# voutcn/megahit

Measured on NVIDIA H100. Metric: sorted (k+1)-mer edges/sec at k=27 on 150bp reads, higher is better.
Workload: dtype u32

## Files before the change

### megahit_b200/csrc/mhb_hashcount.cu

```cuda
#include <cuda_runtime.h>
#include <stdio.h>
#include <string.h>

#include "mhb.h"
#include "mhb_common.cuh"
#include "mhb_count.cuh"

using namespace mhb;

namespace {

constexpr int kHcHist = 1024;
constexpr u64 kHcEmpty = ~0ull;
constexpr int kHcBatch = 4;
constexpr u32 kRemBits = 42;
constexpr u32 kHcHotCount = 256;
constexpr int kHcHotRound = 32;
constexpr int kHcMaxProbes = 48;
constexpr int kHcStack = 72;

__device__ __forceinline__ u64 rec_key64(const uint2 r) { return ((u64)r.x << 32) | r.y; }

__global__ void k_bucket_bounds(const uint2 *__restrict__ recs, u64 n, u64 *__restrict__ bounds) {
  const u32 b = blockIdx.x * blockDim.x + threadIdx.x;
  if (b > 65536u) return;
  u64 lo = 0, hi = n;
  while (lo < hi) {
    const u64 mid = (lo + hi) >> 1;
    if ((recs[mid].x >> 16) < b) lo = mid + 1;
    else hi = mid;
  }
  bounds[b] = lo;
}

template <int THREADS_, int LOG_SLOTS_, int CTAS_>
struct HcGeom {
  static constexpr int THREADS = THREADS_, LOG_SLOTS = LOG_SLOTS_, SLOTS = 1 << LOG_SLOTS_, CTAS = CTAS_;
  static constexpr int MAX_SOLID = SLOTS / 4;
  static constexpr int CELLS = 2 * THREADS;
  static constexpr int LOG_CELLS = LOG_SLOTS_ - 2 >= 0 ? (THREADS_ == 256 ? 9 : (THREADS_ == 512 ? 10 : 11)) : 9;
  static constexpr u32 SLICE = (u32)(SLOTS * 1.83);
};

template <class G>
struct HcShared {
  u64 keys[G::SLOTS];
  u32 cnt[G::SLOTS];
  u32 pt[G::SLOTS];
  u32 nt[G::SLOTS];
  u64 sorted[G::MAX_SOLID];
  u64 tmp[G::MAX_SOLID];
  u32 cell_base[G::CELLS];
  u32 cell_cur[G::CELLS];
  u32 cta_hist[kHcHist];
  u32 wide[kHcHotRound][8];
  uint16_t hot_slot[G::MAX_SOLID];
  u64 st_prefix[kHcStack];
  u32 st_bits[kHcStack];
  u32 warp_sum[G::THREADS / 32];
  u32 n_solid, n_hot, overflow, bucket, out_cursor, sp;
};

__device__ __forceinline__ u32 lane_lt_mask() { return (1u << (threadIdx.x & 31)) - 1u; }

__device__ __forceinline__ void smem_add(u32 *p, u32 v) {
  asm volatile("red.shared.add.u32 [%0], %1;" ::"r"((u32)__cvta_generic_to_shared(p)), "r"(v) : "memory");
}

template <class G>
__device__ __forceinline__ u32 hc_hash(u64 r) { return (u32)((r * 0x9E3779B97F4A7C15ull) >> (64 - G::LOG_SLOTS)); }

template <class G>
__device__ __forceinline__ u32 hc_insert(HcShared<G> &s, u64 r) {
  u32 h = hc_hash<G>(r);
  for (int probes = 0; probes < kHcMaxProbes; ++probes) {
    u64 cur = s.keys[h];
    if (cur == r) return h;
    if (cur == kHcEmpty) {
      cur = atomicCAS((unsigned long long *)&s.keys[h], kHcEmpty, r);
      if (cur == kHcEmpty || cur == r) return h;
    }
    h = (h + 1) & (G::SLOTS - 1);
  }
  return G::SLOTS;
}
template <class G>
__device__ __forceinline__ u32 hc_find(const HcShared<G> &s, u64 r) {
  u32 h = hc_hash<G>(r);
  while (s.keys[h] != r) h = (h + 1) & (G::SLOTS - 1);
  return h;
}

template <class G>
__device__ __forceinline__ void hc_hist_undo(HcShared<G> &s, u64 *mul_hist) {
  for (u32 i = threadIdx.x; i < (u32)G::SLOTS; i += G::THREADS) {
    if (s.keys[i] == kHcEmpty) continue;
    const u32 c = s.cnt[i];
    const u32 c16 = c > 65535u ? 65535u : c;
    if (c16 < (u32)kHcHist) atomicAdd(&s.cta_hist[c16], 0xFFFFFFFFu);
    else atomicAdd((unsigned long long *)&mul_hist[c16], ~0ull);
  }
}

template <class G>
__device__ __forceinline__ void hc_scan_cells(HcShared<G> &s) {
  const u32 t = threadIdx.x, lane = t & 31, w = t >> 5;
  const u32 a = s.cell_base[2 * t], b = s.cell_base[2 * t + 1];
  u32 v = a + b;
#pragma unroll
  for (int d = 1; d < 32; d <<= 1) {
    const u32 o = __shfl_up_sync(0xffffffffu, v, d);
    if ((int)lane >= d) v += o;
  }
  if (lane == 31) s.warp_sum[w] = v;
  __syncthreads();
  if (w == 0) {
    u32 x = lane < G::THREADS / 32 ? s.warp_sum[lane] : 0u;
#pragma unroll
    for (int d = 1; d < 32; d <<= 1) {
      const u32 o = __shfl_up_sync(0xffffffffu, x, d);
      if ((int)lane >= d) x += o;
    }
    if (lane < G::THREADS / 32) s.warp_sum[lane] = x;
  }
  __syncthreads();
  const u32 excl = v - (a + b) + (w ? s.warp_sum[w - 1] : 0u);
  s.cell_base[2 * t] = excl;
  s.cell_base[2 * t + 1] = excl + a;
  s.cell_cur[2 * t] = excl;
  s.cell_cur[2 * t + 1] = excl + a;
  __syncthreads();
}

__device__ __forceinline__ bool hc_any_byte_ge(u32 w, u32 m) {
  return (w & 0xFFu) >= m || ((w >> 8) & 0xFFu) >= m || ((w >> 16) & 0xFFu) >= m || (w >> 24) >= m;
}

template <int THREADS>
__device__ __forceinline__ u64 hc_align(const uint2 *__restrict__ recs, u64 p, u64 lo, u64 hi, u32 *s_min) {
  if (p <= lo) return lo;
  if (p >= hi) return hi;
  for (u64 q0 = p; q0 < hi; q0 += THREADS) {
    __syncthreads();
    if (threadIdx.x == 0) *s_min = 0xFFFFFFFFu;
    __syncthreads();
    const u64 q = q0 + threadIdx.x;
    if (q < hi && (recs[q].x >> 8) != (recs[q - 1].x >> 8)) atomicMin(s_min, threadIdx.x);
    __syncthreads();
    const u32 f = *s_min;
    if (f != 0xFFFFFFFFu) return q0 + f;
  }
  return hi;
}

template <class G>
__global__ void __launch_bounds__(G::THREADS, G::CTAS)
    k_hash_count(const uint2 *__restrict__ recs, const u64 *__restrict__ bounds, const u64 *__restrict__ slice_off,
                 const u64 *__restrict__ n_slices_dev, int m, u32 *ticket, u64 *__restrict__ list,
                 u32 *__restrict__ slice_count, u64 *__restrict__ slice_base, u32 *__restrict__ slice_bucket, u64 *mul_hist,
                 u32 *err_flag) {
  constexpr int THREADS = G::THREADS, SLOTS = G::SLOTS, MAX_SOLID = G::MAX_SOLID, CELLS = G::CELLS;
  extern __shared__ __align__(16) unsigned char smem_raw[];
  HcShared<G> &s = *reinterpret_cast<HcShared<G> *>(smem_raw);
  const u32 tid = threadIdx.x;
  for (u32 i = tid; i < kHcHist; i += THREADS) s.cta_hist[i] = 0;
  for (u32 i = tid; i < (u32)SLOTS; i += THREADS) {
    s.keys[i] = kHcEmpty;
    s.cnt[i] = 0;
    s.pt[i] = 0;
    s.nt[i] = 0;
  }
  __syncthreads();
  const u64 n_slices = *n_slices_dev;
  const u32 um = (u32)m;
  while (true) {
    if (tid == 0) {
      const u32 sl = atomicAdd(ticket, 1u);
      s.bucket = sl;
      if (sl < n_slices) {
        u32 a = 0, z = 65536;
        while (z - a > 1) {
          const u32 mid = (a + z) >> 1;
          if (slice_off[mid] <= sl) a = mid; else z = mid;
        }
        s.sp = a;
      }
    }
    __syncthreads();
    const u32 sl = s.bucket;
    if (sl >= n_slices) break;
    const u32 b = s.sp;
    __syncthreads();
    const u64 blo = bounds[b], bhi = bounds[b + 1];
    const u64 n_in_b = slice_off[b + 1] - slice_off[b], idx = sl - slice_off[b];
    const u64 step = (bhi - blo + n_in_b - 1) / n_in_b;
    const u64 lo = hc_align<THREADS>(recs, blo + idx * step, blo, bhi, &s.overflow);
    const u64 hi = idx + 1 == n_in_b ? bhi : hc_align<THREADS>(recs, blo + (idx + 1) * step, blo, bhi, &s.overflow);
    __syncthreads();
    const u64 base = lo / (u64)m + sl;
    if (tid == 0) {
      slice_base[sl] = base;
      slice_bucket[sl] = b;
      s.out_cursor = 0;
      s.st_prefix[0] = 0;
      s.st_bits[0] = 0;
      s.sp = 1;
    }
    if (hi <= lo) {
      if (tid == 0) slice_count[sl] = 0;
      __syncthreads();
      continue;
    }
    __syncthreads();
    while (s.sp > 0) {
      const u32 sp = s.sp - 1;
      const u64 prefix = s.st_prefix[sp];
      const u32 bits = s.st_bits[sp];
      __syncthreads();
      if (tid == 0) {
        s.sp = sp;
        s.n_solid = 0;
        s.n_hot = 0;
        s.overflow = 0;
      }
      __syncthreads();
      for (u64 i0 = lo + tid; i0 < hi; i0 += (u64)THREADS * kHcBatch) {
        uint2 v[kHcBatch];
#pragma unroll
        for (int j = 0; j < kHcBatch; ++j) {
          const u64 i = i0 + (u64)j * THREADS;
          v[j] = i < hi ? recs[i] : make_uint2(0, 0);
        }
#pragma unroll
        for (int j = 0; j < kHcBatch; ++j) {
          const u64 i = i0 + (u64)j * THREADS;
          if (i >= hi) break;
          const u64 key = rec_key64(v[j]);
          const u64 r = (key >> 6) & ((1ull << kRemBits) - 1);
          if (bits && (r >> (kRemBits - bits)) != prefix) continue;
          const u32 h = hc_insert<G>(s, r);
          if (h == (u32)SLOTS) {
            s.overflow = 1;
            continue;
          }
          smem_add(&s.cnt[h], 1u);
          const u32 p = (u32)(key >> 3) & 7u, nx = (u32)key & 7u;
          if (p < 4) smem_add(&s.pt[h], 1u << (8 * p));
          if (nx < 4) smem_add(&s.nt[h], 1u << (8 * nx));
        }
        if (s.overflow) break;
      }
      __syncthreads();
      bool failed = s.overflow != 0;
      u32 ns = 0;
      if (!failed) {
        for (u32 i0 = 0; i0 < (u32)SLOTS; i0 += THREADS) {
          const u32 slot = i0 + tid;
          const bool on = s.keys[slot] != kHcEmpty;
          const u32 c = on ? s.cnt[slot] : 0u;
          const u32 c16 = c > 65535u ? 65535u : c;
          const u32 ones = __ballot_sync(0xffffffffu, on && c16 == 1u), twos = __ballot_sync(0xffffffffu, on && c16 == 2u);
          if (on && c16 > 2u) {
            if (c16 < (u32)kHcHist) smem_add(&s.cta_hist[c16], 1u);
            else atomicAdd((unsigned long long *)&mul_hist[c16], 1ull);
          }
          const bool solid = on && c >= um;
          const u32 sm_ = __ballot_sync(0xffffffffu, solid);
          u32 wbase = 0;
          if ((tid & 31) == 0) {
            if (ones) atomicAdd(&s.cta_hist[1], (u32)__popc(ones));
            if (twos) atomicAdd(&s.cta_hist[2], (u32)__popc(twos));
            if (sm_) wbase = atomicAdd(&s.n_solid, (u32)__popc(sm_));
          }
          wbase = __shfl_sync(0xffffffffu, wbase, 0);
          if (solid) {
            const u32 rank = wbase + __popc(sm_ & lane_lt_mask());
            if (rank < (u32)MAX_SOLID) {
              u64 e = (s.keys[slot] << 22) | ((u64)c16 << 6);
              if (c >= kHcHotCount) {
                const u32 hi_ = atomicAdd(&s.n_hot, 1u);
                if (hi_ < (u32)MAX_SOLID) s.hot_slot[hi_] = (uint16_t)slot;
                s.pt[slot] = hi_;
                s.nt[slot] = rank;
              } else {
                e |= (hc_any_byte_ge(s.pt[slot], um) ? 0ull : 1ull) | (hc_any_byte_ge(s.nt[slot], um) ? 0ull : 2ull);
              }
              s.sorted[rank] = e;
            }
          }
        }
        __syncthreads();
        ns = s.n_solid;
        if (ns > (u32)MAX_SOLID) {
          hc_hist_undo<G>(s, mul_hist);
          failed = true;
        }
      }
      if (!failed && ns) {
        const u32 n_hot = s.n_hot;
        for (u32 h0 = 0; h0 < n_hot; h0 += kHcHotRound) {
          for (u32 i = tid; i < (u32)kHcHotRound * 8; i += THREADS) s.wide[i >> 3][i & 7] = 0;
          __syncthreads();
          for (u64 i0 = lo + tid; i0 < hi; i0 += (u64)THREADS * kHcBatch) {
            uint2 v[kHcBatch];
#pragma unroll
            for (int j = 0; j < kHcBatch; ++j) {
              const u64 i = i0 + (u64)j * THREADS;
              v[j] = i < hi ? recs[i] : make_uint2(0, 0);
            }
#pragma unroll
            for (int j = 0; j < kHcBatch; ++j) {
              const u64 i = i0 + (u64)j * THREADS;
              if (i >= hi) break;
              const u64 key = rec_key64(v[j]);
              const u64 r = (key >> 6) & ((1ull << kRemBits) - 1);
              if (bits && (r >> (kRemBits - bits)) != prefix) continue;
              const u32 slot = hc_find<G>(s, r);
              const u32 c = s.cnt[slot];
              if (c < kHcHotCount || c < um) continue;
              const u32 hidx = s.pt[slot] - h0;
              if (hidx >= (u32)kHcHotRound) continue;
              const u32 p = (u32)(key >> 3) & 7u, nx = (u32)key & 7u;
              if (p < 4) smem_add(&s.wide[hidx][p], 1u);
              if (nx < 4) smem_add(&s.wide[hidx][4 + nx], 1u);
            }
          }
          __syncthreads();
          for (u32 i = tid; i < (u32)kHcHotRound && h0 + i < n_hot; i += THREADS) {
            bool has_in = false, has_out = false;
#pragma unroll
            for (int c = 0; c < 4; ++c) {
              has_in = has_in || s.wide[i][c] >= um;
              has_out = has_out || s.wide[i][4 + c] >= um;
            }
            s.sorted[s.nt[s.hot_slot[h0 + i]]] |= (has_in ? 0ull : 1ull) | (has_out ? 0ull : 2ull);
          }
          __syncthreads();
        }
        for (u32 i = tid; i < (u32)CELLS; i += THREADS) s.cell_base[i] = 0;
        __syncthreads();
        const u32 cshift = 22 + (kRemBits - G::LOG_CELLS);
        for (u32 i = tid; i < ns; i += THREADS) smem_add(&s.cell_base[(u32)((s.sorted[i] << bits) >> cshift)], 1u);
        __syncthreads();
        hc_scan_cells<G>(s);
        for (u32 i = tid; i < ns; i += THREADS) {
          const u64 e = s.sorted[i];
          s.tmp[atomicAdd(&s.cell_cur[(u32)((e << bits) >> cshift)], 1u)] = e;
        }
        __syncthreads();
        const u32 at = s.out_cursor;
        for (u32 i = tid; i < ns; i += THREADS) {
          const u64 e = s.tmp[i];
          const u32 c = (u32)((e << bits) >> cshift);
          const u32 b0 = s.cell_base[c], b1 = c + 1 < (u32)CELLS ? s.cell_base[c + 1] : ns;
          u32 r = b0;
          for (u32 j = b0; j < b1; ++j) r += s.tmp[j] < e ? 1u : 0u;
          list[base + at + r] = e;
        }
        __syncthreads();
        if (tid == 0) s.out_cursor = at + ns;
      }
      for (u32 i = tid; i < (u32)SLOTS; i += THREADS) {
        s.keys[i] = kHcEmpty;
        s.cnt[i] = 0;
        s.pt[i] = 0;
        s.nt[i] = 0;
      }
      __syncthreads();
      if (tid == 0 && failed) {
        if (bits + 2 > kRemBits || s.sp + 4 > (u32)kHcStack) atomicExch(err_flag, 1u);
        else
          for (int c = 3; c >= 0; --c) {
            s.st_prefix[s.sp] = (prefix << 2) | (u64)c;
            s.st_bits[s.sp] = bits + 2;
            ++s.sp;
          }
      }
      __syncthreads();
    }
    if (tid == 0) slice_count[sl] = s.out_cursor;
    __syncthreads();
  }
  for (u32 i = tid; i < kHcHist; i += THREADS)
    if (s.cta_hist[i]) atomicAdd((unsigned long long *)&mul_hist[i], (unsigned long long)s.cta_hist[i]);
}

using HcGeomA = HcGeom<256, 11, 3>;
using HcGeomB = HcGeom<512, 12, 2>;
using HcGeomC = HcGeom<1024, 13, 1>;

__global__ void k_slice_counts(const u64 *__restrict__ bounds, u32 T, u32 *__restrict__ cnt) {
  const u32 b = blockIdx.x * blockDim.x + threadIdx.x;
  if (b >= 65536u) return;
  const u64 nb = bounds[b + 1] - bounds[b];
  cnt[b] = (u32)((nb + T - 1) / T);
}

__global__ void __launch_bounds__(256)
    k_hash_gather(const u64 *__restrict__ list, const u64 *__restrict__ n_slices_dev, const u32 *__restrict__ slice_count,
                  const u64 *__restrict__ slice_dst, const u64 *__restrict__ slice_base, const u32 *__restrict__ slice_bucket,
                  u32 we, u32 *__restrict__ edges, uint8_t *__restrict__ aux, u64 capacity, const u32 *err_flag,
                  u64 *n_solid_out) {
  const u32 lane = threadIdx.x & 31;
  if (blockIdx.x == 0 && threadIdx.x == 0 && *err_flag) *n_solid_out = ~0ull;
  const u64 n_slices = *n_slices_dev;
  for (u64 sl = (u64)blockIdx.x * 8 + (threadIdx.x >> 5); sl < n_slices; sl += (u64)gridDim.x * 8) {
    const u32 cnt = slice_count[sl];
    if (!cnt) continue;
    const u64 base = slice_base[sl], off = slice_dst[sl], b = slice_bucket[sl];
    for (u32 x = lane; x < cnt; x += 32) {
      if (off + x >= capacity) break;
      const u64 ent = list[base + x];
      const u64 key = (b << 48) | ((ent >> 22) << 6);
      u32 *e = edges + (off + x) * we;
      e[0] = (u32)(key >> 32);
      e[1] = (u32)key;
      if (we == 3) e[2] = 0;
      e[we - 1] |= (u32)(ent >> 6) & 0xFFFFu;
      aux[off + x] = (uint8_t)(ent & 3u);
    }
  }
}

int scan_counts(cudaStream_t st, const u32 *in, u64 n, u64 *out, u64 *total_dev, u64 *bsum) {
  const u64 nb = (n + kScanTile - 1) / kScanTile;
  k_scan32_sums<<<(unsigned)nb, kScanThreads, 0, st>>>(in, n, bsum);
  CK_LAUNCH();
  k_scan_u64<<<1, 1024, 0, st>>>(bsum, nb, total_dev);
  CK_LAUNCH();
  k_scan32_apply<<<(unsigned)nb, kScanThreads, 0, st>>>(in, n, bsum, out);
  CK_LAUNCH();
  return MHB_OK;
}

static int hc_geom() {
  static const int g = getenv("MHB_HC_GEOM") ? (getenv("MHB_HC_GEOM")[0] == 'A' ? 0 : (getenv("MHB_HC_GEOM")[0] == 'C' ? 2 : 1)) : 1;
  return g;
}
static u32 hc_slice_records() {
  const u32 def = hc_geom() == 0 ? HcGeomA::SLICE : (hc_geom() == 1 ? HcGeomB::SLICE : HcGeomC::SLICE);
  static const u32 v = getenv("MHB_HC_SLICE") ? (u32)atoi(getenv("MHB_HC_SLICE")) : 0;
  return v >= 256 && v <= 64000 ? v : def;
}
#define kHcSliceRecords hc_slice_records()

template <class G>
static int launch_hash_count(cudaStream_t st, const uint2 *recs, const u64 *bounds, const u64 *slice_off, const u64 *n_slices_dev,
                             int m, u32 *misc, u64 *list, u32 *slice_count, u64 *slice_base, u32 *slice_bucket, u64 *mul_hist) {
  static int bps = 0;
  const size_t smem = sizeof(HcShared<G>);
  if (!bps) {
    CK(cudaFuncSetAttribute(k_hash_count<G>, cudaFuncAttributeMaxDynamicSharedMemorySize, (int)smem));
    CK(cudaOccupancyMaxActiveBlocksPerMultiprocessor(&bps, k_hash_count<G>, G::THREADS, smem));
    if (bps < 1) return mhb_set_error(MHB_ERR_CUDA, "hash-count kernel does not fit an SM (%zu B shared memory)", smem);
    if (getenv("MHB_VERBOSE")) fprintf(stderr, "[mhb] hash count: %d threads, %d slots, %zu B smem, %d CTA/SM, slice %u\n", G::THREADS, G::SLOTS, smem, bps, kHcSliceRecords);
  }
  k_hash_count<G><<<sm_count() * bps, G::THREADS, smem, st>>>(recs, bounds, slice_off, n_slices_dev, m, misc, list, slice_count,
                                                             slice_base, slice_bucket, mul_hist, misc + 1);
  CK_LAUNCH();
  return MHB_OK;
}

struct HcLayout {
  size_t sort_ws, off_bounds, off_bcnt, off_soff, off_bsum, off_misc, off_scount, off_sdst, off_sbase, off_sbucket, off_list, total;
  uint64_t max_slices;
};
HcLayout hc_layout(uint64_t n, int32_t m) {
  HcLayout L;
  auto pad = [](size_t x) { return (x + 255) & ~(size_t)255; };
  L.max_slices = n / 256 + 65536 + 2;
  L.sort_ws = pad(mhb_sort_workspace_bytes(n, 2));
  size_t p = L.sort_ws;
  L.off_bounds = p;
  p += pad(65537 * 8);
  L.off_bcnt = p;
  p += pad(65537 * 4);
  L.off_soff = p;
  p += pad(65537 * 8);
  L.off_bsum = p;
  p += pad((L.max_slices / kScanTile + 4) * 8);
  L.off_misc = p;
  p += 256;
  L.off_scount = p;
  p += pad(L.max_slices * 4);
  L.off_sdst = p;
  p += pad(L.max_slices * 8);
  L.off_sbase = p;
  p += pad(L.max_slices * 8);
  L.off_sbucket = p;
  p += pad(L.max_slices * 4);
  L.off_list = p;
  p += pad((size_t)(n / (uint64_t)(m < 1 ? 1 : m) + L.max_slices + 8) * 8);
  L.total = p;
  return L;
}

}

extern "C" int mhb_count_hashed_supported(uint32_t k, int32_t m) {
  return count_record_words(k) == 2 && 2 * (k + 1) >= 24 && m >= 1 && m <= kHcHist;
}

extern "C" size_t mhb_count_hashed_workspace_bytes(uint64_t n, uint32_t k, int32_t m) {
  (void)k;
  return hc_layout(n, m).total;
}

extern "C" int mhb_count_solid_hashed(void *stream, uint32_t *recs_a, uint32_t *recs_b, uint64_t n, uint32_t k, int32_t m,
                                      const uint64_t *hist_byte5, uint32_t *edges_out, uint8_t *aux_out,
                                      uint64_t capacity_edges, uint64_t *mul_hist, uint64_t *n_solid_out, void *ws,
                                      size_t ws_bytes) {
  if (!mhb_count_hashed_supported(k, m)) return mhb_set_error(MHB_ERR_ARG, "hashed count needs 8-byte records (11 <= k <= 28) and 1 <= m <= %d", kHcHist);
  if (!mul_hist || !n_solid_out || !ws) return mhb_set_error(MHB_ERR_ARG, "bad args");
  if (n == 0) return MHB_OK;
  if (n >= (1ull << 40)) return mhb_set_error(MHB_ERR_ARG, "too many records for one hashed count call");
  const HcLayout L = hc_layout(n, m);
  if (ws_bytes < L.total) return mhb_set_error(MHB_ERR_ARG, "hashed count workspace too small (%zu < %zu)", ws_bytes, L.total);
  cudaStream_t st = (cudaStream_t)stream;
  const uint8_t bytes[3] = {5, 6, 7};
  int in_b = 0;
  if (int rc = mhb_sort_records_impl(st, recs_a, recs_b, n, 2, bytes, 3, hist_byte5, ws, L.sort_ws, &in_b, nullptr)) return rc;
  const uint2 *recs = (const uint2 *)(in_b ? recs_b : recs_a);
  char *w = (char *)ws;
  u64 *bounds = (u64 *)(w + L.off_bounds);
  u32 *bcnt = (u32 *)(w + L.off_bcnt);
  u64 *slice_off = (u64 *)(w + L.off_soff);
  u64 *bsum = (u64 *)(w + L.off_bsum);
  u32 *misc = (u32 *)(w + L.off_misc);
  u32 *slice_count = (u32 *)(w + L.off_scount);
  u64 *slice_dst = (u64 *)(w + L.off_sdst);
  u64 *slice_base = (u64 *)(w + L.off_sbase);
  u32 *slice_bucket = (u32 *)(w + L.off_sbucket);
  u64 *list = (u64 *)(w + L.off_list);
  u64 *n_slices_dev = (u64 *)(misc + 2);
  CK(cudaMemsetAsync(misc, 0, 256, st));
  CK(cudaMemsetAsync(slice_count, 0, L.max_slices * 4, st));
  k_bucket_bounds<<<(65537 + 255) / 256, 256, 0, st>>>(recs, n, bounds);
  CK_LAUNCH();
  k_slice_counts<<<65536 / 256, 256, 0, st>>>(bounds, kHcSliceRecords, bcnt);
  CK_LAUNCH();
  if (int rc = scan_counts(st, bcnt, 65536, slice_off, n_slices_dev, bsum)) return rc;
  CK(cudaMemcpyAsync(slice_off + 65536, n_slices_dev, 8, cudaMemcpyDeviceToDevice, st));
  {
    int rc;
    if (hc_geom() == 0) rc = launch_hash_count<HcGeomA>(st, recs, bounds, slice_off, n_slices_dev, m, misc, list, slice_count, slice_base, slice_bucket, mul_hist);
    else if (hc_geom() == 2) rc = launch_hash_count<HcGeomC>(st, recs, bounds, slice_off, n_slices_dev, m, misc, list, slice_count, slice_base, slice_bucket, mul_hist);
    else rc = launch_hash_count<HcGeomB>(st, recs, bounds, slice_off, n_slices_dev, m, misc, list, slice_count, slice_base, slice_bucket, mul_hist);
    if (rc) return rc;
  }
  if (int rc = scan_counts(st, slice_count, L.max_slices, slice_dst, n_solid_out, bsum)) return rc;
  k_hash_gather<<<sm_count() * 4, 256, 0, st>>>(list, n_slices_dev, slice_count, slice_dst, slice_base, slice_bucket,
                                               words_per_edge(k), edges_out, aux_out, capacity_edges, misc + 1, n_solid_out);
  CK_LAUNCH();
  return MHB_OK;
}
```

Measured before the change: 13.68 billion.

## Precompute slice plan, prefetch next slice to L2, and streamline hash-count loop

Slice boundary alignment moves out of the hash-count kernel into a separate per-bucket planning kernel that uses binary search. The count kernel now reads precomputed ranges, fetches the next ticket early and issues bulk L2 prefetches for the next slice while the current one is processed. Table clearing is folded into the extraction pass, and cell histogramming moves into solid extraction. Hot-key passes use a small rehash, the histogram-undo pass is dropped in favour of a done flag on the stack, the batch size doubles, and the alternative geometries and env knobs are removed. The aim is fewer block-wide syncs and less memory latency, but the kernel is more complex and register pressure may rise.

```diff
diff --git a/megahit_b200/csrc/mhb_hashcount.cu b/megahit_b200/csrc/mhb_hashcount.cu
--- a/megahit_b200/csrc/mhb_hashcount.cu
+++ b/megahit_b200/csrc/mhb_hashcount.cu
@@ -12,12 +12,14 @@
 
 constexpr int kHcHist = 1024;
 constexpr u64 kHcEmpty = ~0ull;
-constexpr int kHcBatch = 4;
+constexpr int kHcBatch = 8;
 constexpr u32 kRemBits = 42;
 constexpr u32 kHcHotCount = 256;
 constexpr int kHcHotRound = 32;
 constexpr int kHcMaxProbes = 48;
 constexpr int kHcStack = 72;
+constexpr u32 kHcHistDone = 1u << 31;
+constexpr u32 kHcPrefetchChunk = 16384;
 
 __device__ __forceinline__ u64 rec_key64(const uint2 r) { return ((u64)r.x << 32) | r.y; }
 
@@ -31,6 +33,36 @@
     else hi = mid;
   }
   bounds[b] = lo;
+}
+
+__device__ __forceinline__ u64 hc_align(const uint2 *__restrict__ recs, u64 p, u64 lo, u64 hi) {
+  if (p <= lo) return lo;
+  if (p >= hi) return hi;
+  const u32 pre = recs[p - 1].x >> 8;
+  u64 a = p, z = hi;
+  while (a < z) {
+    const u64 mid = (a + z) >> 1;
+    if ((recs[mid].x >> 8) > pre) z = mid;
+    else a = mid + 1;
+  }
+  return a;
+}
+
+__global__ void k_slice_plan(const uint2 *__restrict__ recs, const u64 *__restrict__ bounds, const u64 *__restrict__ slice_off,
+                             int m, ulonglong2 *__restrict__ plan, u64 *__restrict__ slice_base, u32 *__restrict__ slice_bucket) {
+  const u32 b = blockIdx.x * blockDim.x + threadIdx.x;
+  if (b >= 65536u) return;
+  const u64 s0 = slice_off[b], ns = slice_off[b + 1] - s0;
+  if (!ns) return;
+  const u64 blo = bounds[b], bhi = bounds[b + 1], step = (bhi - blo + ns - 1) / ns;
+  u64 lo = blo;
+  for (u64 i = 0; i < ns; ++i) {
+    const u64 hi = i + 1 == ns ? bhi : hc_align(recs, blo + (i + 1) * step, blo, bhi);
+    plan[s0 + i] = make_ulonglong2(lo, hi);
+    slice_base[s0 + i] = lo / (u64)m + s0 + i;
+    slice_bucket[s0 + i] = b;
+    lo = hi;
+  }
 }
 
 template <int THREADS_, int LOG_SLOTS_, int CTAS_>
@@ -54,17 +86,27 @@
   u32 cell_cur[G::CELLS];
   u32 cta_hist[kHcHist];
   u32 wide[kHcHotRound][8];
-  uint16_t hot_slot[G::MAX_SOLID];
+  uint16_t hot_rank[G::MAX_SOLID];
   u64 st_prefix[kHcStack];
   u32 st_bits[kHcStack];
   u32 warp_sum[G::THREADS / 32];
-  u32 n_solid, n_hot, overflow, bucket, out_cursor, sp;
+  ulonglong2 nx_range[2];
+  u32 nx_sl[2];
+  u32 n_solid[2], n_hot[2], overflow[2];
 };
 
 __device__ __forceinline__ u32 lane_lt_mask() { return (1u << (threadIdx.x & 31)) - 1u; }
 
 __device__ __forceinline__ void smem_add(u32 *p, u32 v) {
   asm volatile("red.shared.add.u32 [%0], %1;" ::"r"((u32)__cvta_generic_to_shared(p)), "r"(v) : "memory");
+}
+
+__device__ __forceinline__ void hc_prefetch_l2(const uint2 *recs, u64 lo, u64 hi) {
+  const u64 a0 = (u64)(recs + lo) & ~15ull, a1 = (u64)(recs + hi) & ~15ull;
+  for (u64 a = a0; a < a1; a += kHcPrefetchChunk) {
+    const u32 sz = (u32)(a1 - a < kHcPrefetchChunk ? a1 - a : kHcPrefetchChunk);
+    asm volatile("cp.async.bulk.prefetch.L2.global [%0], %1;" ::"l"(a), "r"(sz) : "memory");
+  }
 }
 
 template <class G>
@@ -85,27 +127,20 @@
   return G::SLOTS;
 }
 template <class G>
-__device__ __forceinline__ u32 hc_find(const HcShared<G> &s, u64 r) {
+__device__ __forceinline__ u32 hc_lookup(const HcShared<G> &s, u64 r) {
   u32 h = hc_hash<G>(r);
-  while (s.keys[h] != r) h = (h + 1) & (G::SLOTS - 1);
-  return h;
-}
-
-template <class G>
-__device__ __forceinline__ void hc_hist_undo(HcShared<G> &s, u64 *mul_hist) {
-  for (u32 i = threadIdx.x; i < (u32)G::SLOTS; i += G::THREADS) {
-    if (s.keys[i] == kHcEmpty) continue;
-    const u32 c = s.cnt[i];
-    const u32 c16 = c > 65535u ? 65535u : c;
-    if (c16 < (u32)kHcHist) atomicAdd(&s.cta_hist[c16], 0xFFFFFFFFu);
-    else atomicAdd((unsigned long long *)&mul_hist[c16], ~0ull);
+  while (true) {
+    const u64 cur = s.keys[h];
+    if (cur == r) return h;
+    if (cur == kHcEmpty) return G::SLOTS;
+    h = (h + 1) & (G::SLOTS - 1);
   }
 }
 
 template <class G>
 __device__ __forceinline__ void hc_scan_cells(HcShared<G> &s) {
   const u32 t = threadIdx.x, lane = t & 31, w = t >> 5;
-  const u32 a = s.cell_base[2 * t], b = s.cell_base[2 * t + 1];
+  const u32 a = s.cell_cur[2 * t], b = s.cell_cur[2 * t + 1];
   u32 v = a + b;
 #pragma unroll
   for (int d = 1; d < 32; d <<= 1) {
@@ -136,94 +171,74 @@
   return (w & 0xFFu) >= m || ((w >> 8) & 0xFFu) >= m || ((w >> 16) & 0xFFu) >= m || (w >> 24) >= m;
 }
 
-template <int THREADS>
-__device__ __forceinline__ u64 hc_align(const uint2 *__restrict__ recs, u64 p, u64 lo, u64 hi, u32 *s_min) {
-  if (p <= lo) return lo;
-  if (p >= hi) return hi;
-  for (u64 q0 = p; q0 < hi; q0 += THREADS) {
-    __syncthreads();
-    if (threadIdx.x == 0) *s_min = 0xFFFFFFFFu;
-    __syncthreads();
-    const u64 q = q0 + threadIdx.x;
-    if (q < hi && (recs[q].x >> 8) != (recs[q - 1].x >> 8)) atomicMin(s_min, threadIdx.x);
-    __syncthreads();
-    const u32 f = *s_min;
-    if (f != 0xFFFFFFFFu) return q0 + f;
-  }
-  return hi;
-}
-
 template <class G>
 __global__ void __launch_bounds__(G::THREADS, G::CTAS)
-    k_hash_count(const uint2 *__restrict__ recs, const u64 *__restrict__ bounds, const u64 *__restrict__ slice_off,
-                 const u64 *__restrict__ n_slices_dev, int m, u32 *ticket, u64 *__restrict__ list,
-                 u32 *__restrict__ slice_count, u64 *__restrict__ slice_base, u32 *__restrict__ slice_bucket, u64 *mul_hist,
-                 u32 *err_flag) {
+    k_hash_count(const uint2 *__restrict__ recs, const ulonglong2 *__restrict__ plan, const u64 *__restrict__ n_slices_dev,
+                 int m, u32 *ticket, u64 *__restrict__ list, u32 *__restrict__ slice_count, u64 *mul_hist, u32 *err_flag) {
   constexpr int THREADS = G::THREADS, SLOTS = G::SLOTS, MAX_SOLID = G::MAX_SOLID, CELLS = G::CELLS;
   extern __shared__ __align__(16) unsigned char smem_raw[];
   HcShared<G> &s = *reinterpret_cast<HcShared<G> *>(smem_raw);
   const u32 tid = threadIdx.x;
   for (u32 i = tid; i < kHcHist; i += THREADS) s.cta_hist[i] = 0;
+  for (u32 i = tid; i < (u32)CELLS; i += THREADS) s.cell_cur[i] = 0;
   for (u32 i = tid; i < (u32)SLOTS; i += THREADS) {
     s.keys[i] = kHcEmpty;
     s.cnt[i] = 0;
     s.pt[i] = 0;
     s.nt[i] = 0;
   }
-  __syncthreads();
   const u64 n_slices = *n_slices_dev;
   const u32 um = (u32)m;
-  while (true) {
-    if (tid == 0) {
-      const u32 sl = atomicAdd(ticket, 1u);
-      s.bucket = sl;
-      if (sl < n_slices) {
-        u32 a = 0, z = 65536;
-        while (z - a > 1) {
-          const u32 mid = (a + z) >> 1;
-          if (slice_off[mid] <= sl) a = mid; else z = mid;
-        }
-        s.sp = a;
+  const u32 cshift = 22 + (kRemBits - G::LOG_CELLS);
+  u32 tk = 0;
+  if (tid == 0) {
+    s.n_solid[0] = s.n_solid[1] = s.n_hot[0] = s.n_hot[1] = s.overflow[0] = s.overflow[1] = 0;
+    const u32 t0 = atomicAdd(ticket, 1u);
+    s.nx_sl[0] = t0;
+    if (t0 < n_slices) {
+      const ulonglong2 r = plan[t0];
+      s.nx_range[0] = r;
+      hc_prefetch_l2(recs, r.x, r.y);
+      tk = atomicAdd(ticket, 1u);
+    } else {
+      tk = t0;
+    }
+  }
+  __syncthreads();
+  u32 q = 0;
+  for (u32 it = 0;; ++it) {
+    const u32 sl = s.nx_sl[it & 1];
+    if (sl >= n_slices) break;
+    const ulonglong2 rg = s.nx_range[it & 1];
+    const u64 lo = rg.x, hi = rg.y;
+    ulonglong2 nx = make_ulonglong2(0, 0);
+    u32 ntk = tk;
+    if (tid == 0 && tk < n_slices) {
+      nx = plan[tk];
+      ntk = atomicAdd(ticket, 1u);
+    }
+    auto publish_next = [&]() {
+      if (tid != 0) return;
+      s.nx_sl[(it + 1) & 1] = tk;
+      if (tk < n_slices) {
+        s.nx_range[(it + 1) & 1] = nx;
+        hc_prefetch_l2(recs, nx.x, nx.y);
       }
-    }
-    __syncthreads();
-    const u32 sl = s.bucket;
-    if (sl >= n_slices) break;
-    const u32 b = s.sp;
-    __syncthreads();
-    const u64 blo = bounds[b], bhi = bounds[b + 1];
-    const u64 n_in_b = slice_off[b + 1] - slice_off[b], idx = sl - slice_off[b];
-    const u64 step = (bhi - blo + n_in_b - 1) / n_in_b;
-    const u64 lo = hc_align<THREADS>(recs, blo + idx * step, blo, bhi, &s.overflow);
-    const u64 hi = idx + 1 == n_in_b ? bhi : hc_align<THREADS>(recs, blo + (idx + 1) * step, blo, bhi, &s.overflow);
-    __syncthreads();
-    const u64 base = lo / (u64)m + sl;
-    if (tid == 0) {
-      slice_base[sl] = base;
-      slice_bucket[sl] = b;
-      s.out_cursor = 0;
-      s.st_prefix[0] = 0;
-      s.st_bits[0] = 0;
-      s.sp = 1;
-    }
+      tk = ntk;
+    };
     if (hi <= lo) {
-      if (tid == 0) slice_count[sl] = 0;
+      publish_next();
       __syncthreads();
       continue;
     }
-    __syncthreads();
-    while (s.sp > 0) {
-      const u32 sp = s.sp - 1;
-      const u64 prefix = s.st_prefix[sp];
-      const u32 bits = s.st_bits[sp];
-      __syncthreads();
-      if (tid == 0) {
-        s.sp = sp;
-        s.n_solid = 0;
-        s.n_hot = 0;
-        s.overflow = 0;
-      }
-      __syncthreads();
+    const u64 base = lo / (u64)m + sl;
+    u32 out_cursor = 0, sp = 0;
+    u64 prefix = 0;
+    u32 bits = 0;
+    bool hist_done = false, first = true;
+    while (true) {
+      const u32 par = q & 1;
+      ++q;
       for (u64 i0 = lo + tid; i0 < hi; i0 += (u64)THREADS * kHcBatch) {
         uint2 v[kHcBatch];
 #pragma unroll
@@ -240,154 +255,169 @@
           if (bits && (r >> (kRemBits - bits)) != prefix) continue;
           const u32 h = hc_insert<G>(s, r);
           if (h == (u32)SLOTS) {
-            s.overflow = 1;
+            s.overflow[par] = 1;
             continue;
           }
           smem_add(&s.cnt[h], 1u);
-          const u32 p = (u32)(key >> 3) & 7u, nx = (u32)key & 7u;
+          const u32 p = (u32)(key >> 3) & 7u, nx_ = (u32)key & 7u;
           if (p < 4) smem_add(&s.pt[h], 1u << (8 * p));
-          if (nx < 4) smem_add(&s.nt[h], 1u << (8 * nx));
-        }
-        if (s.overflow) break;
+          if (nx_ < 4) smem_add(&s.nt[h], 1u << (8 * nx_));
+        }
+        if (s.overflow[par]) break;
       }
+      if (first) publish_next();
+      first = false;
       __syncthreads();
-      bool failed = s.overflow != 0;
-      u32 ns = 0;
-      if (!failed) {
-        for (u32 i0 = 0; i0 < (u32)SLOTS; i0 += THREADS) {
-          const u32 slot = i0 + tid;
-          const bool on = s.keys[slot] != kHcEmpty;
-          const u32 c = on ? s.cnt[slot] : 0u;
-          const u32 c16 = c > 65535u ? 65535u : c;
+      const bool overflowed = s.overflow[par] != 0;
+      if (tid == 0) s.n_solid[par ^ 1] = s.n_hot[par ^ 1] = s.overflow[par ^ 1] = 0;
+      const bool count_hist = !overflowed && !hist_done;
+      for (u32 slot = tid; slot < (u32)SLOTS; slot += THREADS) {
+        const u64 key = s.keys[slot];
+        const bool on = key != kHcEmpty;
+        u32 c = 0, ptv = 0, ntv = 0;
+        if (on) {
+          c = s.cnt[slot];
+          ptv = s.pt[slot];
+          ntv = s.nt[slot];
+          s.keys[slot] = kHcEmpty;
+          s.cnt[slot] = 0;
+          s.pt[slot] = 0;
+          s.nt[slot] = 0;
+        }
+        if (overflowed) continue;
+        const u32 c16 = c > 65535u ? 65535u : c;
+        if (count_hist) {
           const u32 ones = __ballot_sync(0xffffffffu, on && c16 == 1u), twos = __ballot_sync(0xffffffffu, on && c16 == 2u);
           if (on && c16 > 2u) {
             if (c16 < (u32)kHcHist) smem_add(&s.cta_hist[c16], 1u);
             else atomicAdd((unsigned long long *)&mul_hist[c16], 1ull);
           }
-          const bool solid = on && c >= um;
-          const u32 sm_ = __ballot_sync(0xffffffffu, solid);
-          u32 wbase = 0;
           if ((tid & 31) == 0) {
-            if (ones) atomicAdd(&s.cta_hist[1], (u32)__popc(ones));
-            if (twos) atomicAdd(&s.cta_hist[2], (u32)__popc(twos));
-            if (sm_) wbase = atomicAdd(&s.n_solid, (u32)__popc(sm_));
-          }
-          wbase = __shfl_sync(0xffffffffu, wbase, 0);
-          if (solid) {
-            const u32 rank = wbase + __popc(sm_ & lane_lt_mask());
-            if (rank < (u32)MAX_SOLID) {
-              u64 e = (s.keys[slot] << 22) | ((u64)c16 << 6);
-              if (c >= kHcHotCount) {
-                const u32 hi_ = atomicAdd(&s.n_hot, 1u);
-                if (hi_ < (u32)MAX_SOLID) s.hot_slot[hi_] = (uint16_t)slot;
-                s.pt[slot] = hi_;
-                s.nt[slot] = rank;
-              } else {
-                e |= (hc_any_byte_ge(s.pt[slot], um) ? 0ull : 1ull) | (hc_any_byte_ge(s.nt[slot], um) ? 0ull : 2ull);
+            if (ones) smem_add(&s.cta_hist[1], (u32)__popc(ones));
+            if (twos) smem_add(&s.cta_hist[2], (u32)__popc(twos));
+          }
+        }
+        const bool solid = on && c >= um;
+        const u32 sm_ = __ballot_sync(0xffffffffu, solid);
+        if (!sm_) continue;
+        u32 wbase = 0;
+        if ((tid & 31) == 0) wbase = atomicAdd(&s.n_solid[par], (u32)__popc(sm_));
+        wbase = __shfl_sync(0xffffffffu, wbase, 0);
+        if (solid) {
+          const u32 rank = wbase + __popc(sm_ & lane_lt_mask());
+          if (rank < (u32)MAX_SOLID) {
+            u64 e = (key << 22) | ((u64)c16 << 6);
+            if (c >= kHcHotCount) {
+              s.hot_rank[atomicAdd(&s.n_hot[par], 1u)] = (uint16_t)rank;
+            } else {
+              e |= (hc_any_byte_ge(ptv, um) ? 0ull : 1ull) | (hc_any_byte_ge(ntv, um) ? 0ull : 2ull);
+            }
+            s.sorted[rank] = e;
+            smem_add(&s.cell_cur[(u32)((e << bits) >> cshift)], 1u);
+          }
+        }
+      }
+      __syncthreads();
+      const u32 ns = s.n_solid[par];
+      const bool failed = overflowed || ns > (u32)MAX_SOLID;
+      if (!failed && ns) {
+        const u32 n_hot = s.n_hot[par];
+        if (n_hot) {
+          for (u32 i = tid; i < n_hot; i += THREADS) {
+            const u64 r = s.sorted[s.hot_rank[i]] >> 22;
+            u32 h = hc_hash<G>(r);
+            while (atomicCAS((unsigned long long *)&s.keys[h], kHcEmpty, r) != kHcEmpty) h = (h + 1) & (SLOTS - 1);
+            s.pt[h] = i;
+          }
+          for (u32 h0 = 0; h0 < n_hot; h0 += kHcHotRound) {
+            for (u32 i = tid; i < (u32)kHcHotRound * 8; i += THREADS) s.wide[i >> 3][i & 7] = 0;
+            __syncthreads();
+            for (u64 i0 = lo + tid; i0 < hi; i0 += (u64)THREADS * kHcBatch) {
+              uint2 v[kHcBatch];
+#pragma unroll
+              for (int j = 0; j < kHcBatch; ++j) {
+                const u64 i = i0 + (u64)j * THREADS;
+                v[j] = i < hi ? recs[i] : make_uint2(0, 0);
               }
-              s.sorted[rank] = e;
+#pragma unroll
+              for (int j = 0; j < kHcBatch; ++j) {
+                const u64 i = i0 + (u64)j * THREADS;
+                if (i >= hi) break;
+                const u64 key = rec_key64(v[j]);
+                const u64 r = (key >> 6) & ((1ull << kRemBits) - 1);
+                if (bits && (r >> (kRemBits - bits)) != prefix) continue;
+                const u32 slot = hc_lookup<G>(s, r);
+                if (slot == (u32)SLOTS) continue;
+                const u32 hidx = s.pt[slot] - h0;
+                if (hidx >= (u32)kHcHotRound) continue;
+                const u32 p = (u32)(key >> 3) & 7u, nx_ = (u32)key & 7u;
+                if (p < 4) smem_add(&s.wide[hidx][p], 1u);
+                if (nx_ < 4) smem_add(&s.wide[hidx][4 + nx_], 1u);
+              }
             }
-          }
-        }
-        __syncthreads();
-        ns = s.n_solid;
-        if (ns > (u32)MAX_SOLID) {
-          hc_hist_undo<G>(s, mul_hist);
-          failed = true;
-        }
-      }
-      if (!failed && ns) {
-        const u32 n_hot = s.n_hot;
-        for (u32 h0 = 0; h0 < n_hot; h0 += kHcHotRound) {
-          for (u32 i = tid; i < (u32)kHcHotRound * 8; i += THREADS) s.wide[i >> 3][i & 7] = 0;
-          __syncthreads();
-          for (u64 i0 = lo + tid; i0 < hi; i0 += (u64)THREADS * kHcBatch) {
-            uint2 v[kHcBatch];
-#pragma unroll
-            for (int j = 0; j < kHcBatch; ++j) {
-              const u64 i = i0 + (u64)j * THREADS;
-              v[j] = i < hi ? recs[i] : make_uint2(0, 0);
+            __syncthreads();
+            for (u32 i = tid; i < (u32)kHcHotRound && h0 + i < n_hot; i += THREADS) {
+              bool has_in = false, has_out = false;
+#pragma unroll
+              for (int c = 0; c < 4; ++c) {
+                has_in = has_in || s.wide[i][c] >= um;
+                has_out = has_out || s.wide[i][4 + c] >= um;
+              }
+              s.sorted[s.hot_rank[h0 + i]] |= (has_in ? 0ull : 1ull) | (has_out ? 0ull : 2ull);
             }
-#pragma unroll
-            for (int j = 0; j < kHcBatch; ++j) {
-              const u64 i = i0 + (u64)j * THREADS;
-              if (i >= hi) break;
-              const u64 key = rec_key64(v[j]);
-              const u64 r = (key >> 6) & ((1ull << kRemBits) - 1);
-              if (bits && (r >> (kRemBits - bits)) != prefix) continue;
-              const u32 slot = hc_find<G>(s, r);
-              const u32 c = s.cnt[slot];
-              if (c < kHcHotCount || c < um) continue;
-              const u32 hidx = s.pt[slot] - h0;
-              if (hidx >= (u32)kHcHotRound) continue;
-              const u32 p = (u32)(key >> 3) & 7u, nx = (u32)key & 7u;
-              if (p < 4) smem_add(&s.wide[hidx][p], 1u);
-              if (nx < 4) smem_add(&s.wide[hidx][4 + nx], 1u);
-            }
-          }
-          __syncthreads();
-          for (u32 i = tid; i < (u32)kHcHotRound && h0 + i < n_hot; i += THREADS) {
-            bool has_in = false, has_out = false;
-#pragma unroll
-            for (int c = 0; c < 4; ++c) {
-              has_in = has_in || s.wide[i][c] >= um;
-              has_out = has_out || s.wide[i][4 + c] >= um;
-            }
-            s.sorted[s.nt[s.hot_slot[h0 + i]]] |= (has_in ? 0ull : 1ull) | (has_out ? 0ull : 2ull);
-          }
-          __syncthreads();
-        }
-        for (u32 i = tid; i < (u32)CELLS; i += THREADS) s.cell_base[i] = 0;
-        __syncthreads();
-        const u32 cshift = 22 + (kRemBits - G::LOG_CELLS);
-        for (u32 i = tid; i < ns; i += THREADS) smem_add(&s.cell_base[(u32)((s.sorted[i] << bits) >> cshift)], 1u);
-        __syncthreads();
+            __syncthreads();
+          }
+          for (u32 i = tid; i < (u32)SLOTS; i += THREADS) {
+            s.keys[i] = kHcEmpty;
+            s.pt[i] = 0;
+          }
+        }
         hc_scan_cells<G>(s);
         for (u32 i = tid; i < ns; i += THREADS) {
           const u64 e = s.sorted[i];
           s.tmp[atomicAdd(&s.cell_cur[(u32)((e << bits) >> cshift)], 1u)] = e;
         }
         __syncthreads();
-        const u32 at = s.out_cursor;
+        for (u32 i = tid; i < (u32)CELLS; i += THREADS) s.cell_cur[i] = 0;
         for (u32 i = tid; i < ns; i += THREADS) {
           const u64 e = s.tmp[i];
           const u32 c = (u32)((e << bits) >> cshift);
           const u32 b0 = s.cell_base[c], b1 = c + 1 < (u32)CELLS ? s.cell_base[c + 1] : ns;
           u32 r = b0;
           for (u32 j = b0; j < b1; ++j) r += s.tmp[j] < e ? 1u : 0u;
-          list[base + at + r] = e;
+          list[base + out_cursor + r] = e;
+        }
+        out_cursor += ns;
+      }
+      if (failed) {
+        for (u32 i = tid; i < (u32)CELLS; i += THREADS) s.cell_cur[i] = 0;
+        if (bits + 2 > kRemBits || sp + 4 > (u32)kHcStack) {
+          if (tid == 0) atomicExch(err_flag, 1u);
+        } else {
+          const u32 flag = (hist_done || !overflowed) ? kHcHistDone : 0u;
+          if (tid == 0)
+            for (int c = 3; c >= 0; --c) {
+              s.st_prefix[sp + 3 - c] = (prefix << 2) | (u64)c;
+              s.st_bits[sp + 3 - c] = (bits + 2) | flag;
+            }
+          sp += 4;
         }
         __syncthreads();
-        if (tid == 0) s.out_cursor = at + ns;
       }
-      for (u32 i = tid; i < (u32)SLOTS; i += THREADS) {
-        s.keys[i] = kHcEmpty;
-        s.cnt[i] = 0;
-        s.pt[i] = 0;
-        s.nt[i] = 0;
-      }
-      __syncthreads();
-      if (tid == 0 && failed) {
-        if (bits + 2 > kRemBits || s.sp + 4 > (u32)kHcStack) atomicExch(err_flag, 1u);
-        else
-          for (int c = 3; c >= 0; --c) {
-            s.st_prefix[s.sp] = (prefix << 2) | (u64)c;
-            s.st_bits[s.sp] = bits + 2;
-            ++s.sp;
-          }
-      }
-      __syncthreads();
-    }
-    if (tid == 0) slice_count[sl] = s.out_cursor;
-    __syncthreads();
-  }
+      if (sp == 0) break;
+      --sp;
+      prefix = s.st_prefix[sp];
+      bits = s.st_bits[sp] & ~kHcHistDone;
+      hist_done = (s.st_bits[sp] & kHcHistDone) != 0;
+    }
+    if (tid == 0) slice_count[sl] = out_cursor;
+  }
+  __syncthreads();
   for (u32 i = tid; i < kHcHist; i += THREADS)
     if (s.cta_hist[i]) atomicAdd((unsigned long long *)&mul_hist[i], (unsigned long long)s.cta_hist[i]);
 }
 
-using HcGeomA = HcGeom<256, 11, 3>;
 using HcGeomB = HcGeom<512, 12, 2>;
-using HcGeomC = HcGeom<1024, 13, 1>;
 
 __global__ void k_slice_counts(const u64 *__restrict__ bounds, u32 T, u32 *__restrict__ cnt) {
   const u32 b = blockIdx.x * blockDim.x + threadIdx.x;
@@ -433,42 +463,32 @@
   return MHB_OK;
 }
 
-static int hc_geom() {
-  static const int g = getenv("MHB_HC_GEOM") ? (getenv("MHB_HC_GEOM")[0] == 'A' ? 0 : (getenv("MHB_HC_GEOM")[0] == 'C' ? 2 : 1)) : 1;
-  return g;
-}
-static u32 hc_slice_records() {
-  const u32 def = hc_geom() == 0 ? HcGeomA::SLICE : (hc_geom() == 1 ? HcGeomB::SLICE : HcGeomC::SLICE);
-  static const u32 v = getenv("MHB_HC_SLICE") ? (u32)atoi(getenv("MHB_HC_SLICE")) : 0;
-  return v >= 256 && v <= 64000 ? v : def;
-}
-#define kHcSliceRecords hc_slice_records()
-
-template <class G>
-static int launch_hash_count(cudaStream_t st, const uint2 *recs, const u64 *bounds, const u64 *slice_off, const u64 *n_slices_dev,
-                             int m, u32 *misc, u64 *list, u32 *slice_count, u64 *slice_base, u32 *slice_bucket, u64 *mul_hist) {
+template <class G>
+static int launch_hash_count(cudaStream_t st, const uint2 *recs, const ulonglong2 *plan, const u64 *n_slices_dev, int m, u32 *misc,
+                             u64 *list, u32 *slice_count, u64 *mul_hist) {
   static int bps = 0;
   const size_t smem = sizeof(HcShared<G>);
   if (!bps) {
     CK(cudaFuncSetAttribute(k_hash_count<G>, cudaFuncAttributeMaxDynamicSharedMemorySize, (int)smem));
     CK(cudaOccupancyMaxActiveBlocksPerMultiprocessor(&bps, k_hash_count<G>, G::THREADS, smem));
     if (bps < 1) return mhb_set_error(MHB_ERR_CUDA, "hash-count kernel does not fit an SM (%zu B shared memory)", smem);
-    if (getenv("MHB_VERBOSE")) fprintf(stderr, "[mhb] hash count: %d threads, %d slots, %zu B smem, %d CTA/SM, slice %u\n", G::THREADS, G::SLOTS, smem, bps, kHcSliceRecords);
-  }
-  k_hash_count<G><<<sm_count() * bps, G::THREADS, smem, st>>>(recs, bounds, slice_off, n_slices_dev, m, misc, list, slice_count,
-                                                             slice_base, slice_bucket, mul_hist, misc + 1);
+    if (getenv("MHB_VERBOSE")) fprintf(stderr, "[mhb] hash count: %d threads, %d slots, %zu B smem, %d CTA/SM, slice %u\n", G::THREADS, G::SLOTS, smem, bps, G::SLICE);
+  }
+  k_hash_count<G><<<sm_count() * bps, G::THREADS, smem, st>>>(recs, plan, n_slices_dev, m, misc, list, slice_count, mul_hist,
+                                                             misc + 1);
   CK_LAUNCH();
   return MHB_OK;
 }
 
 struct HcLayout {
-  size_t sort_ws, off_bounds, off_bcnt, off_soff, off_bsum, off_misc, off_scount, off_sdst, off_sbase, off_sbucket, off_list, total;
+  size_t sort_ws, off_bounds, off_bcnt, off_soff, off_bsum, off_misc, off_scount, off_sdst, off_sbase, off_sbucket, off_plan,
+      off_list, total;
   uint64_t max_slices;
 };
 HcLayout hc_layout(uint64_t n, int32_t m) {
   HcLayout L;
   auto pad = [](size_t x) { return (x + 255) & ~(size_t)255; };
-  L.max_slices = n / 256 + 65536 + 2;
+  L.max_slices = n / HcGeomB::SLICE + 65536 + 2;
   L.sort_ws = pad(mhb_sort_workspace_bytes(n, 2));
   size_t p = L.sort_ws;
   L.off_bounds = p;
@@ -489,6 +509,8 @@
   p += pad(L.max_slices * 8);
   L.off_sbucket = p;
   p += pad(L.max_slices * 4);
+  L.off_plan = p;
+  p += pad(L.max_slices * 16);
   L.off_list = p;
   p += pad((size_t)(n / (uint64_t)(m < 1 ? 1 : m) + L.max_slices + 8) * 8);
   L.total = p;
@@ -531,23 +553,20 @@
   u64 *slice_dst = (u64 *)(w + L.off_sdst);
   u64 *slice_base = (u64 *)(w + L.off_sbase);
   u32 *slice_bucket = (u32 *)(w + L.off_sbucket);
+  ulonglong2 *plan = (ulonglong2 *)(w + L.off_plan);
   u64 *list = (u64 *)(w + L.off_list);
   u64 *n_slices_dev = (u64 *)(misc + 2);
   CK(cudaMemsetAsync(misc, 0, 256, st));
   CK(cudaMemsetAsync(slice_count, 0, L.max_slices * 4, st));
   k_bucket_bounds<<<(65537 + 255) / 256, 256, 0, st>>>(recs, n, bounds);
   CK_LAUNCH();
-  k_slice_counts<<<65536 / 256, 256, 0, st>>>(bounds, kHcSliceRecords, bcnt);
+  k_slice_counts<<<65536 / 256, 256, 0, st>>>(bounds, HcGeomB::SLICE, bcnt);
   CK_LAUNCH();
   if (int rc = scan_counts(st, bcnt, 65536, slice_off, n_slices_dev, bsum)) return rc;
   CK(cudaMemcpyAsync(slice_off + 65536, n_slices_dev, 8, cudaMemcpyDeviceToDevice, st));
-  {
-    int rc;
-    if (hc_geom() == 0) rc = launch_hash_count<HcGeomA>(st, recs, bounds, slice_off, n_slices_dev, m, misc, list, slice_count, slice_base, slice_bucket, mul_hist);
-    else if (hc_geom() == 2) rc = launch_hash_count<HcGeomC>(st, recs, bounds, slice_off, n_slices_dev, m, misc, list, slice_count, slice_base, slice_bucket, mul_hist);
-    else rc = launch_hash_count<HcGeomB>(st, recs, bounds, slice_off, n_slices_dev, m, misc, list, slice_count, slice_base, slice_bucket, mul_hist);
-    if (rc) return rc;
-  }
+  k_slice_plan<<<65536 / 256, 256, 0, st>>>(recs, bounds, slice_off, m, plan, slice_base, slice_bucket);
+  CK_LAUNCH();
+  if (int rc = launch_hash_count<HcGeomB>(st, recs, plan, n_slices_dev, m, misc, list, slice_count, mul_hist)) return rc;
   if (int rc = scan_counts(st, slice_count, L.max_slices, slice_dst, n_solid_out, bsum)) return rc;
   k_hash_gather<<<sm_count() * 4, 256, 0, st>>>(list, n_slices_dev, slice_count, slice_dst, slice_base, slice_bucket,
                                                words_per_edge(k), edges_out, aux_out, capacity_edges, misc + 1, n_solid_out);
```

Measured after the change: 14.19 billion, median of 6. 1.04x the previous value.
